# czbiohub-sf/shrimPy

Hardware: AMD Instinct MI355X
Metric: voxels/sec deskew+20-iter RL deconv, 2048×2048×512 f32; HBM GB/s vs peak (higher is better)
Workload: dtype f32

## Files before the change

### shrimpy_amd/csrc/rl_fused_sep.hip

```cpp

#include "common.hpp"
#include "correlate_common.hpp"

#ifndef LSR_FUSED_PZ
#error "compile with -DLSR_FUSED_PZ=<odd tap count along z>"
#endif

namespace {

using lsr::FusedArgs;

constexpr int kTX = lsr::kSepWideTileX;
constexpr int kWaves = 8;
constexpr int kThreads = 64 * kWaves;
constexpr int kBand = 8;
constexpr int kRing = 3;

constexpr int cdiv(int a, int b) { return (a + b - 1) / b; }

template <int PZ, int PYX, int RUN>
struct Geo {
  static constexpr int C = PYX / 2, CZ = PZ / 2;
  static constexpr int TY = 8 * RUN;
  static constexpr int WL = lsr::fused_window_halo(PYX);
  static constexpr int AR = TY + 4 * C;
  static constexpr int PA = kTX + 2 * WL;
  static constexpr int CH = PA / 4;
  static constexpr int NCH = AR * CH;
  static constexpr int SL = cdiv(NCH, kThreads);
  static constexpr int ASZ = cdiv(NCH, 64) * 64 * 4;
  static constexpr int NP = cdiv(4 + 2 * C, 4);
  static constexpr int G1 = (kTX + WL) / 4;
  static constexpr int PB1 = 4 * G1;
  static constexpr int NIT1 = AR * G1;
  static constexpr int XIT1 = cdiv(NIT1, kThreads);
  static constexpr int R1 = TY + 2 * C;
  static constexpr int RUN1 = cdiv(R1, 8);
  static constexpr int E = PB1 - kTX;
  static constexpr int NE = R1 * E;
  static constexpr int EP = cdiv(NE, kThreads);
  static constexpr int SH = WL - 2 * C;
  static constexpr int PR = 4 * (kTX / 4 - 1 + NP);
  static constexpr int RSZ = 4 + 8 * RUN1 * PR;
  static constexpr int NIT2 = R1 * (kTX / 4);
  static constexpr int XIT2 = cdiv(NIT2, kThreads);
  static constexpr int B1SZ = AR * PB1;
  static constexpr int B2SZ = R1 * kTX;
  static constexpr int OFF_B1 = kRing * ASZ;
  static constexpr int OFF_R = OFF_B1 + B1SZ;
  static constexpr int OFF_B2 = OFF_R + RSZ;
  static constexpr int OFF_DUMP = OFF_B2 + B2SZ;
  static constexpr int OFF_RNY = OFF_DUMP + 256;
  static constexpr int TOTAL = OFF_RNY + 32;
  static constexpr int NY = 2 * RUN1 + EP;
#ifdef LSR_FUSED_PROBE_NOXC
  static constexpr int NXC = 0;
#else
  static constexpr int NXC = 2 * RUN + 1;
#endif
  static_assert(TOTAL * 4 <= 160 * 1024, "LDS per workgroup");
  static_assert(PR == PB1, "B1 and R share a pitch");
  static_assert(2 * C <= WL && WL <= lsr::kSepOriginCol, "halo columns");
  static_assert(SL + 2 * (NY + NXC) <= 63, "vmcnt is a 6-bit counter");
  static_assert(OFF_B1 % 4 == 0 && OFF_R % 4 == 0 && OFF_B2 % 4 == 0, "16-byte aligned buffers");
};

typedef float f32x4 __attribute__((ext_vector_type(4)));
typedef float f32x2 __attribute__((ext_vector_type(2)));

__device__ __forceinline__ float fast_rcp(float d) {
  float r = __builtin_amdgcn_rcpf(d);
  return fmaf(fmaf(-d, r, 1.0f), r, r);
}
__device__ __forceinline__ f32x2 splat(float a) { return f32x2{a, a}; }
__device__ __forceinline__ f32x2 pk_fma(f32x2 a, f32x2 b, f32x2 c) { return __builtin_elementwise_fma(a, b, c); }
__device__ __forceinline__ f32x2 fast_rcp2(f32x2 d) {
  const f32x2 r = f32x2{__builtin_amdgcn_rcpf(d.x), __builtin_amdgcn_rcpf(d.y)};
  return pk_fma(pk_fma(-d, r, splat(1.0f)), r, r);
}
template <int PX, int NP>
__device__ __forceinline__ f32x4 xpass_item(const f32x4* src, const float (&wx)[PX]) {
  float w[4 * NP];
#pragma unroll
  for (int i = 0; i < NP; ++i) {
    const f32x4 v = src[i];
    w[4 * i] = v.x; w[4 * i + 1] = v.y; w[4 * i + 2] = v.z; w[4 * i + 3] = v.w;
  }
  f32x2 o01 = splat(wx[0]) * f32x2{w[0], w[1]};
  f32x2 o23 = splat(wx[0]) * f32x2{w[2], w[3]};
#pragma unroll
  for (int c = 1; c < PX; ++c) {
    o01 = pk_fma(splat(wx[c]), f32x2{w[c], w[c + 1]}, o01);
    o23 = pk_fma(splat(wx[c]), f32x2{w[c + 2], w[c + 3]}, o23);
  }
  return f32x4{o01.x, o01.y, o23.x, o23.y};
}

template <int IMM>
__device__ __forceinline__ void gload(float& dst, const float* sbase, int voff) {
  asm volatile("global_load_dword %0, %1, %2 offset:%3" : "+v"(dst) : "v"(voff), "s"(sbase), "n"(IMM) : "memory");
}
#ifndef LSR_FUSED_STORE_POLICY
#define LSR_FUSED_STORE_POLICY "nt"
#endif
#ifndef LSR_FUSED_GLDS_POLICY
#define LSR_FUSED_GLDS_POLICY ""
#endif
template <int IMM>
__device__ __forceinline__ void gstore(float* sbase, int voff, float v) {
  asm volatile("global_store_dword %0, %1, %2 offset:%3 " LSR_FUSED_STORE_POLICY
               :
               : "v"(voff), "v"(v), "s"(sbase), "n"(IMM)
               : "memory");
}
__device__ __forceinline__ void glds_x4(const float* sbase, int voff, unsigned lds_byte_addr) {
  asm volatile("s_mov_b32 m0, %2\n\ts_nop 0\n\tglobal_load_lds_dwordx4 %0, %1 " LSR_FUSED_GLDS_POLICY
               :
               : "v"(voff), "s"(sbase), "s"(lds_byte_addr)
               : "memory");
}
template <int N>
__device__ __forceinline__ void wait_vm() {
  asm volatile("s_waitcnt vmcnt(%0)" : : "n"(N) : "memory");
}
template <int K>
__device__ __forceinline__ void tie(float (&a)[K]) {
#pragma unroll
  for (int i = 0; i < K; ++i) asm volatile("" : "+v"(a[i]));
}
__device__ __forceinline__ void tie(float& a) { asm volatile("" : "+v"(a)); }
__device__ __forceinline__ void lds_barrier() {
  asm volatile("s_waitcnt lgkmcnt(0)" ::: "memory");
  __builtin_amdgcn_s_barrier();
  __builtin_amdgcn_sched_barrier(0);
}

template <int PZ, int PYX, int RUN, bool STATS>
__global__ __launch_bounds__(kThreads) void rl_fused_sep_kernel(FusedArgs p) {
  using T = Geo<PZ, PYX, RUN>;
  constexpr int C = T::C, CZ = T::CZ, TY = T::TY, RUN1 = T::RUN1, EP = T::EP;
  constexpr int NP = T::NP, NY = T::NY, NXC = T::NXC, SL = T::SL;
  __shared__ f32x4 smem4[T::TOTAL / 4];
  float* const smem = reinterpret_cast<float*>(smem4);
  f32x4* const B1_4 = smem4 + T::OFF_B1 / 4;
  const float* const B1 = smem + T::OFF_B1;
  float* const Rw = smem + T::OFF_R + 4;
  const f32x4* const R_4 = smem4 + T::OFF_R / 4 + 1;
  f32x4* const B2_4 = smem4 + T::OFF_B2 / 4;
  const float* const B2 = smem + T::OFF_B2;
  const unsigned lds_base =
      static_cast<unsigned>(reinterpret_cast<size_t>((__attribute__((address_space(3))) char*)smem4));

  const int tid = threadIdx.x;
  const int lane = tid & 63;
  const int wave = __builtin_amdgcn_readfirstlane(tid >> 6);

  auto xcd_contiguous = [](int b, int n) {
#ifdef LSR_FUSED_PLAIN_ORDER
    return b;
#endif
    const int per = n / 8, rem = n % 8;
    const int xcd = b % 8, idx = b / 8;
    return xcd * per + (xcd < rem ? xcd : rem) + idx;
  };
  const int Z = p.Z, Y = p.Y, X = p.X;
  int lin, zb, ze;
  if (static_cast<int>(blockIdx.x) < p.n_full) {
    lin = xcd_contiguous(blockIdx.x, p.n_full);
    zb = 0;
    ze = Z;
  } else {
    const int t = xcd_contiguous(blockIdx.x - p.n_full, gridDim.x - p.n_full);
    const int col = t / p.pieces;
    lin = p.n_full + col;
    zb = (t - col * p.pieces) * p.z_chunk;
    ze = min(zb + p.z_chunk, Z);
  }
  const int band = lin / (p.tiles_x * kBand);
  const int lb = lin - band * (p.tiles_x * kBand);
  const int band_h = min(kBand, p.tiles_y - band * kBand);
#if defined(LSR_FUSED_PLAIN_ORDER) && LSR_FUSED_PLAIN_ORDER == 2
  const int tx = lin % p.tiles_x;
  const int ty = lin / p.tiles_x;
  (void)lb; (void)band_h;
#else
  const int tx = lb / band_h;
  const int ty = band * kBand + (lb - tx * band_h);
#endif
  const int x0 = tx * kTX, y0 = ty * TY;
#ifdef LSR_FUSED_LAG
  if ((tx + ty) & 1) {
#pragma unroll
    for (int i = 0; i < LSR_FUSED_LAG; ++i) __builtin_amdgcn_s_sleep(127);
  }
#endif

  float tv0 = p.taps[lane], tv1 = p.taps[64 + (lane & 31)];
  auto load_taps = [&](int row, auto& w) {
#pragma unroll
    for (int i = 0; i < static_cast<int>(sizeof(w) / sizeof(float)); ++i) {
      const int f = row * 16 + i;
      w[i] = __int_as_float(__builtin_amdgcn_readlane(__float_as_int(f < 64 ? tv0 : tv1), f & 63));
    }
  };

  const float* const x_tile = p.x + (static_cast<int64_t>(y0 - 2 * C) * p.pitch + (x0 - T::WL));
  int s_voff[SL];
#pragma unroll
  for (int k = 0; k < SL; ++k) {
    const int e = min(tid + k * kThreads, T::NCH - 1);
    const int r = e / T::CH, c = e - r * T::CH;
    s_voff[k] = (r * p.pitch + 4 * c) * 4;
  }
  int a1_chunk[T::XIT1];
#pragma unroll
  for (int k = 0; k < T::XIT1; ++k) {
    const int i = min(tid + k * kThreads, T::NIT1 - 1);
    const int row = i / T::G1;
    a1_chunk[k] = i + row * (T::CH - T::G1);
  }
  const int r1_row0 = wave * RUN1;
  const int y1_col = r1_row0 * T::PB1 + lane;
  const int r_col = r1_row0 * T::PR + lane - T::SH;
  const bool interior = x0 - C >= 0 && x0 + kTX + C <= X && y0 - C >= 0 && y0 + TY + C <= Y;
  int e_b1[EP], e_voff[EP];
  int e_rc[EP];
#pragma unroll
  for (int e = 0; e < EP; ++e) {
    const int t = min(tid + e * kThreads, T::NE - 1);
    const int er = t / T::E, ec = t - er * T::E;
    e_b1[e] = er * T::PB1 + kTX + ec;
    e_rc[e] = (er << 16) | (kTX + ec);
    e_voff[e] = (er * p.y_pitch + kTX + ec) * 4;
  }
  const int y2_col = (wave * RUN) * kTX + lane;
  int xc_voff[RUN], o_voff[RUN], y_voff[RUN1];
#pragma unroll
  for (int m = 0; m < RUN; ++m) {
    xc_voff[m] = ((wave * RUN + m) * p.pitch + lane) * 4;
    o_voff[m] = ((wave * RUN + m) * p.out_pitch + lane) * 4;
  }
#pragma unroll
  for (int m = 0; m < RUN1; ++m) y_voff[m] = (min(r1_row0 + m, T::R1 - 1) * p.y_pitch + lane) * 4;
  float rnx[2];
#pragma unroll
  for (int cg = 0; cg < 2; ++cg) rnx[cg] = fast_rcp(p.nx[min(x0 + lane + 64 * cg, X - 1)]);
  float* const rny_lds = smem + T::OFF_RNY;
  if (tid < TY) rny_lds[tid] = fast_rcp(p.ny[min(y0 + tid, Y - 1)]);

  f32x2 acc1[PZ][RUN1], acc2[PZ][RUN];
  float acc1e[PZ][EP];
#pragma unroll
  for (int j = 0; j < PZ; ++j) {
#pragma unroll
    for (int i = 0; i < RUN1; ++i) acc1[j][i] = splat(0.0f);
#pragma unroll
    for (int i = 0; i < EP; ++i) acc1e[j][i] = 0.0f;
#pragma unroll
    for (int i = 0; i < RUN; ++i) acc2[j][i] = splat(0.0f);
  }
  float yv[2 * RUN1], ye[EP], xc[2 * RUN], nzv = 1.0f;
#pragma unroll
  for (int i = 0; i < 2 * RUN1; ++i) yv[i] = 0.0f;
#pragma unroll
  for (int i = 0; i < EP; ++i) ye[i] = 0.0f;
#pragma unroll
  for (int i = 0; i < 2 * RUN; ++i) xc[i] = 0.0f;
  const f32x2 rnx2 = f32x2{rnx[0], rnx[1]};
  f32x2 st_flux = splat(0.0f), st_total = splat(0.0f);
  float st_change = 0.0f;
  auto st_add = [&](f32x2 x_old, f32x2 xu, f32x2 v) {
    st_flux += xu;
    st_total += v;
    const f32x2 d = v - x_old;
    st_change += __builtin_fabsf(d.x);
    st_change += __builtin_fabsf(d.y);
  };
  __builtin_amdgcn_sched_barrier(0);

  auto clampz = [&](int z) { return min(max(z, 0), Z - 1); };
  auto issue_glds = [&](int plane, int slot) {
    const float* src = x_tile + static_cast<int64_t>(clampz(plane)) * p.plane;
    const unsigned dst = lds_base + (slot * T::ASZ + wave * 64 * 4) * 4;
#pragma unroll
    for (int k = 0; k < SL; ++k) {
      const bool live = wave * 64 + k * kThreads < T::NCH;
      glds_x4(src, s_voff[k], live ? dst + k * kThreads * 16 : lds_base + T::OFF_DUMP * 4);
    }
  };
  const float* const xc_tile = p.x + (static_cast<int64_t>(y0) * p.pitch + x0);
  const float* const y_tile = p.y + (static_cast<int64_t>(y0 - C) * p.y_pitch + (x0 + C - T::WL));
  float* const o_tile = p.out + (static_cast<int64_t>(y0) * p.out_pitch + x0);
  auto issue_xc = [&](int o) {
#ifdef LSR_FUSED_PROBE_NOXC
    return;
#endif
    const int oc = clampz(o);
    const float* base = xc_tile + static_cast<int64_t>(oc) * p.plane;
#pragma unroll
    for (int m = 0; m < RUN; ++m) {
      gload<0>(xc[m], base, xc_voff[m]);
      gload<256>(xc[RUN + m], base, xc_voff[m]);
    }
    gload<0>(nzv, p.nz + oc, 0);
  };
  auto issue_y = [&](int q) {
    const float* base = y_tile + static_cast<int64_t>(clampz(q)) * p.y_plane;
#pragma unroll
    for (int m = 0; m < RUN1; ++m) {
      gload<0>(yv[m], base, y_voff[m]);
      gload<256>(yv[RUN1 + m], base, y_voff[m]);
    }
#pragma unroll
    for (int e = 0; e < EP; ++e) gload<0>(ye[e], base, e_voff[e]);
  };

  const int q_lo = max(zb - CZ, 0), q_hi = min(ze - 1 + CZ, Z - 1);
  const int p_lo = max(q_lo - CZ, 0);
  const int p_hi = ze + 2 * CZ;

  int slot = 0;
  issue_glds(p_lo, 0);
  issue_xc(p_lo - 1 - 2 * CZ);
  issue_y(p_lo - CZ);
  issue_glds(p_lo + 1, 1);
  issue_xc(p_lo - 1 - 2 * CZ);
  issue_y(p_lo - CZ);
  wait_vm<SL + 2 * (NXC + NY)>();
  lds_barrier();

#ifdef LSR_FUSED_PROBE_TIME
  if (p.probe && tid == 0) p.probe[4 * blockIdx.x] = wall_clock64();
#endif
  for (int pz = p_lo; pz <= p_hi; ++pz) {
    asm volatile("" : "+v"(tv0), "+v"(tv1));
#ifdef LSR_FUSED_PROBE_TIME
    if (p.probe && tid == 0 && (pz == p_lo + 40 || pz == p_lo + 120))
      p.probe[4 * blockIdx.x + (pz == p_lo + 40 ? 1 : 2)] = wall_clock64();
#endif
    const int qr = pz - 1 - CZ;
    const int o = qr - CZ;
    const int q = pz - CZ;
    const bool x_live = pz < Z && pz <= q_hi + CZ;
    const bool r_live = qr >= q_lo && qr <= q_hi;
    const int slot2 = slot >= 1 ? slot - 1 : 2;

    issue_glds(pz + 2, slot2);
#ifdef LSR_FUSED_PROBE_NOCOMPUTE
    if (false) {
#else
    if (x_live) {
#endif
      float w1x[PYX];
      load_taps(0, w1x);
      const f32x4* A_4 = smem4 + slot * (T::ASZ / 4);
#pragma unroll
      for (int k = 0; k < T::XIT1; ++k)
        if (k + 1 < T::XIT1 || tid + k * kThreads < T::NIT1)
          B1_4[tid + k * kThreads] = xpass_item<PYX, NP>(A_4 + a1_chunk[k], w1x);
    } else {
#pragma unroll
      for (int k = 0; k < T::XIT1; ++k)
        if (k + 1 < T::XIT1 || tid + k * kThreads < T::NIT1) B1_4[tid + k * kThreads] = f32x4{0, 0, 0, 0};
    }
#ifdef LSR_FUSED_PROBE_NOCOMPUTE
    if (false) {
#else
    if (r_live) {
#endif
      float w2x[PYX];
      load_taps(3, w2x);
#pragma unroll
      for (int k = 0; k < T::XIT2; ++k) {
        const int j = tid + k * kThreads;
        if (k + 1 < T::XIT2 || j < T::NIT2)
          B2_4[j] = xpass_item<PYX, NP>(R_4 + (j + (j >> 5) * (T::PR / 4 - kTX / 4)), w2x);
      }
    } else {
#pragma unroll
      for (int k = 0; k < T::XIT2; ++k)
        if (k + 1 < T::XIT2 || tid + k * kThreads < T::NIT2) B2_4[tid + k * kThreads] = f32x4{0, 0, 0, 0};
    }
    lds_barrier();

    {
      float w2y[PYX], w2z[PZ];
      load_taps(4, w2y);
      load_taps(5, w2z);
      f32x2 pl[RUN];
#ifdef LSR_FUSED_PROBE_NOCOMPUTE
#pragma unroll
      for (int m = 0; m < RUN; ++m) pl[m] = splat(B2[y2_col + m]);
      if (false)
#endif
      {
        const float* colp = B2 + y2_col;
        f32x2 cv[RUN + 2 * C];
#pragma unroll
        for (int j = 0; j < RUN + 2 * C; ++j) cv[j] = f32x2{colp[j * kTX], colp[j * kTX + 64]};
#pragma unroll
        for (int m = 0; m < RUN; ++m) {
          f32x2 s2 = splat(w2y[0]) * cv[m];
#pragma unroll
          for (int b = 1; b < PYX; ++b) s2 = pk_fma(splat(w2y[b]), cv[m + b], s2);
          pl[m] = s2;
        }
      }
#pragma unroll
      for (int j = 0; j < PZ - 1; ++j)
#pragma unroll
        for (int i = 0; i < RUN; ++i) acc2[j][i] = pk_fma(splat(w2z[PZ - 1 - j]), pl[i], acc2[j + 1][i]);
#pragma unroll
      for (int i = 0; i < RUN; ++i) acc2[PZ - 1][i] = splat(w2z[0]) * pl[i];

      wait_vm<NY + SL>();
      tie(xc);
      tie(nzv);
#ifdef LSR_FUSED_PROBE_NOSTORE
      if (o >= zb && o < ze && nzv == 12345.678f) {
#else
      if (o >= zb && o < ze) {
#endif
        float* obase = o_tile + static_cast<int64_t>(o) * p.out_plane;
        const float rz = fast_rcp(nzv);
        if (!p.mask_out) {
#pragma unroll
          for (int m = 0; m < RUN; ++m) {
            const f32x2 xo = f32x2{xc[m], xc[RUN + m]};
            const f32x2 xu = xo * acc2[0][m];
            const f32x2 v = xu * (splat(rz * rny_lds[wave * RUN + m]) * rnx2);
            gstore<0>(obase, o_voff[m], v.x);
            gstore<256>(obase, o_voff[m], v.y);
            if constexpr (STATS) st_add(xo, xu, v);
          }
        } else {
          const bool ok0 = x0 + lane < X, ok1 = x0 + lane + 64 < X;
#pragma unroll
          for (int m = 0; m < RUN; ++m) {
            if (y0 + wave * RUN + m < Y) {
              const f32x2 xo = f32x2{xc[m], xc[RUN + m]};
              const f32x2 xu = xo * acc2[0][m];
              const f32x2 v = xu * (splat(rz * rny_lds[wave * RUN + m]) * rnx2);
              if (ok0) gstore<0>(obase, o_voff[m], v.x);
              if (ok1) gstore<256>(obase, o_voff[m], v.y);
              if constexpr (STATS) {
                st_add(xo, xu, v);
              }
            }
          }
        }
      }
      __builtin_amdgcn_sched_barrier(0);
      issue_xc(o + 1);
    }
    {
      float w1y[PYX], w1z[PZ];
      load_taps(1, w1y);
      load_taps(2, w1z);
      f32x2 pl[RUN1];
      float ple[EP];
#ifdef LSR_FUSED_PROBE_NOCOMPUTE
#pragma unroll
      for (int m = 0; m < RUN1; ++m) pl[m] = splat(B1[y1_col + m]);
      if (false)
#endif
      {
        const float* colp = B1 + y1_col;
        f32x2 cv[RUN1 + 2 * C];
#pragma unroll
        for (int j = 0; j < RUN1 + 2 * C; ++j) cv[j] = f32x2{colp[j * T::PB1], colp[j * T::PB1 + 64]};
#pragma unroll
        for (int m = 0; m < RUN1; ++m) {
          f32x2 s2 = splat(w1y[0]) * cv[m];
#pragma unroll
          for (int b = 1; b < PYX; ++b) s2 = pk_fma(splat(w1y[b]), cv[m + b], s2);
          pl[m] = s2;
        }
      }
#pragma unroll
      for (int e = 0; e < EP; ++e) {
        const float* colp = B1 + e_b1[e];
#ifdef LSR_FUSED_PROBE_NOCOMPUTE
        ple[e] = colp[0];
        continue;
#endif
        float s1 = w1y[0] * colp[0];
#pragma unroll
        for (int b = 1; b < PYX; ++b) s1 = fmaf(w1y[b], colp[b * T::PB1], s1);
        ple[e] = s1;
      }
#pragma unroll
      for (int j = 0; j < PZ - 1; ++j) {
#pragma unroll
        for (int i = 0; i < RUN1; ++i) acc1[j][i] = pk_fma(splat(w1z[PZ - 1 - j]), pl[i], acc1[j + 1][i]);
#pragma unroll
        for (int e = 0; e < EP; ++e) acc1e[j][e] = fmaf(w1z[PZ - 1 - j], ple[e], acc1e[j + 1][e]);
      }
#pragma unroll
      for (int i = 0; i < RUN1; ++i) acc1[PZ - 1][i] = splat(w1z[0]) * pl[i];
#pragma unroll
      for (int e = 0; e < EP; ++e) acc1e[PZ - 1][e] = w1z[0] * ple[e];

      wait_vm<SL + NXC>();
      tie(yv);
      tie(ye);
      const bool q_in = q >= q_lo && q <= q_hi;
      if (q_in && interior) {
#pragma unroll
        for (int m = 0; m < RUN1; ++m) {
          const f32x2 r = f32x2{yv[m], yv[RUN1 + m]} * fast_rcp2(acc1[0][m] + splat(p.eps));
          Rw[r_col + m * T::PR] = r.x;
          Rw[r_col + m * T::PR + 64] = r.y;
        }
#pragma unroll
        for (int e = 0; e < EP; ++e)
          if (e + 1 < EP || tid + e * kThreads < T::NE)
            Rw[e_b1[e] - T::SH] = ye[e] * fast_rcp(acc1e[0][e] + p.eps);
      } else {
        const int gx0 = x0 + lane + C - T::WL;
        const bool in0 = q_in && gx0 >= 0 && gx0 < X, in1 = q_in && gx0 + 64 >= 0 && gx0 + 64 < X;
#pragma unroll
        for (int m = 0; m < RUN1; ++m) {
          const int gy = y0 + r1_row0 + m - C;
          const bool row_in = gy >= 0 && gy < Y && r1_row0 + m < T::R1;
          const f32x2 r = f32x2{yv[m], yv[RUN1 + m]} * fast_rcp2(acc1[0][m] + splat(p.eps));
          Rw[r_col + m * T::PR] = (row_in && in0) ? r.x : 0.0f;
          Rw[r_col + m * T::PR + 64] = (row_in && in1) ? r.y : 0.0f;
        }
#pragma unroll
        for (int e = 0; e < EP; ++e) {
          if (e + 1 < EP || tid + e * kThreads < T::NE) {
            const int gy = y0 + (e_rc[e] >> 16) - C, gx = x0 + (e_rc[e] & 0xffff) + C - T::WL;
            const float r = ye[e] * fast_rcp(acc1e[0][e] + p.eps);
            Rw[e_b1[e] - T::SH] = (q_in && gy >= 0 && gy < Y && gx >= 0 && gx < X) ? r : 0.0f;
          }
        }
      }
      __builtin_amdgcn_sched_barrier(0);
      issue_y(q + 1);
    }
    wait_vm<SL + 2 * (NXC + NY)>();
    lds_barrier();
    slot = slot == 2 ? 0 : slot + 1;
  }
  asm volatile("s_waitcnt vmcnt(0)" ::: "memory");
  if constexpr (STATS) {
    lsr::keep_until_here(xc);
    lsr::keep_until_here(yv);
    lsr::keep_until_here(ye);
    lsr::keep_until_here(nzv);
    asm volatile("" : "+v"(st_flux), "+v"(st_total), "+v"(st_change));
    lsr::RlStats st;
    st.flux = st_flux.x + st_flux.y;
    st.change = st_change;
    st.total = st_total.x + st_total.y;
    lsr::rl_stats_flush<kWaves>(st, smem + T::OFF_B2, p.stats);
  }
#ifdef LSR_FUSED_PROBE_TIME
  if (p.probe && tid == 0) p.probe[4 * blockIdx.x + 3] = wall_clock64();
#endif
}

template <int PZ, int PYX>
bool launch_one(const FusedArgs& p, dim3 grid, hipStream_t s) {
  if constexpr (lsr::fused_compiled(PZ, PYX)) {
    constexpr int RUN = lsr::fused_run(PZ, PYX);
    if (p.stats != nullptr) hipLaunchKernelGGL((rl_fused_sep_kernel<PZ, PYX, RUN, true>), grid, dim3(kThreads), 0, s, p);
    else hipLaunchKernelGGL((rl_fused_sep_kernel<PZ, PYX, RUN, false>), grid, dim3(kThreads), 0, s, p);
    return true;
  } else {
    return false;
  }
}

}

namespace lsr {

#define LSR_CAT2(a, b) a##b
#define LSR_CAT(a, b) LSR_CAT2(a, b)
bool LSR_CAT(launch_fused_pz, LSR_FUSED_PZ)(int pyx, const FusedArgs& p, unsigned blocks, hipStream_t s) {
  constexpr int PZ = LSR_FUSED_PZ;
  const dim3 grid(blocks);
  switch (pyx) {
    case 3: return launch_one<PZ, 3>(p, grid, s);
    case 5: return launch_one<PZ, 5>(p, grid, s);
    case 7: return launch_one<PZ, 7>(p, grid, s);
    case 9: return launch_one<PZ, 9>(p, grid, s);
    case 11: return launch_one<PZ, 11>(p, grid, s);
    case 13: return launch_one<PZ, 13>(p, grid, s);
    case 15: return launch_one<PZ, 15>(p, grid, s);
    default: return false;
  }
}

}
```

Before: 41.27 billion.

## Load filter taps via scalar constant loads and specialize mask path at compile time

Replaces the per-lane tap vectors fetched with readlane by scalar loads through the constant address space. This frees two VGPRs per thread and moves tap fetches to the scalar unit, with the loads hoisted before the LDS barriers so their latency overlaps. The mask_out branch becomes a template parameter, removing a runtime branch and doubling the number of kernel instantiations. The glds liveness check is also simplified so only the last chunk is predicated.

```diff
diff --git a/shrimpy_amd/csrc/rl_fused_sep.hip b/shrimpy_amd/csrc/rl_fused_sep.hip
--- a/shrimpy_amd/csrc/rl_fused_sep.hip
+++ b/shrimpy_amd/csrc/rl_fused_sep.hip
@@ -135,7 +135,7 @@
   __builtin_amdgcn_sched_barrier(0);
 }
 
-template <int PZ, int PYX, int RUN, bool STATS>
+template <int PZ, int PYX, int RUN, bool STATS, bool MASK>
 __global__ __launch_bounds__(kThreads) void rl_fused_sep_kernel(FusedArgs p) {
   using T = Geo<PZ, PYX, RUN>;
   constexpr int C = T::C, CZ = T::CZ, TY = T::TY, RUN1 = T::RUN1, EP = T::EP;
@@ -195,13 +195,12 @@
   }
 #endif
 
-  float tv0 = p.taps[lane], tv1 = p.taps[64 + (lane & 31)];
+  typedef const __attribute__((address_space(4))) float* ctaps_t;
+  const float* taps = p.taps;
   auto load_taps = [&](int row, auto& w) {
-#pragma unroll
-    for (int i = 0; i < static_cast<int>(sizeof(w) / sizeof(float)); ++i) {
-      const int f = row * 16 + i;
-      w[i] = __int_as_float(__builtin_amdgcn_readlane(__float_as_int(f < 64 ? tv0 : tv1), f & 63));
-    }
+    const ctaps_t t = (ctaps_t)taps;
+#pragma unroll
+    for (int i = 0; i < static_cast<int>(sizeof(w) / sizeof(float)); ++i) w[i] = t[row * 16 + i];
   };
 
   const float* const x_tile = p.x + (static_cast<int64_t>(y0 - 2 * C) * p.pitch + (x0 - T::WL));
@@ -284,7 +283,7 @@
     const unsigned dst = lds_base + (slot * T::ASZ + wave * 64 * 4) * 4;
 #pragma unroll
     for (int k = 0; k < SL; ++k) {
-      const bool live = wave * 64 + k * kThreads < T::NCH;
+      const bool live = k + 1 < SL || wave * 64 + k * kThreads < T::NCH;
       glds_x4(src, s_voff[k], live ? dst + k * kThreads * 16 : lds_base + T::OFF_DUMP * 4);
     }
   };
@@ -332,8 +331,11 @@
 #ifdef LSR_FUSED_PROBE_TIME
   if (p.probe && tid == 0) p.probe[4 * blockIdx.x] = wall_clock64();
 #endif
+  float w1x[PYX], w2x[PYX];
+  load_taps(0, w1x);
+  load_taps(3, w2x);
   for (int pz = p_lo; pz <= p_hi; ++pz) {
-    asm volatile("" : "+v"(tv0), "+v"(tv1));
+    asm volatile("" : "+s"(taps));
 #ifdef LSR_FUSED_PROBE_TIME
     if (p.probe && tid == 0 && (pz == p_lo + 40 || pz == p_lo + 120))
       p.probe[4 * blockIdx.x + (pz == p_lo + 40 ? 1 : 2)] = wall_clock64();
@@ -351,8 +353,6 @@
 #else
     if (x_live) {
 #endif
-      float w1x[PYX];
-      load_taps(0, w1x);
       const f32x4* A_4 = smem4 + slot * (T::ASZ / 4);
 #pragma unroll
       for (int k = 0; k < T::XIT1; ++k)
@@ -368,8 +368,6 @@
 #else
     if (r_live) {
 #endif
-      float w2x[PYX];
-      load_taps(3, w2x);
 #pragma unroll
       for (int k = 0; k < T::XIT2; ++k) {
         const int j = tid + k * kThreads;
@@ -381,12 +379,14 @@
       for (int k = 0; k < T::XIT2; ++k)
         if (k + 1 < T::XIT2 || tid + k * kThreads < T::NIT2) B2_4[tid + k * kThreads] = f32x4{0, 0, 0, 0};
     }
+    float w2y[PYX], w2z[PZ], w1y[PYX], w1z[PZ];
+    load_taps(4, w2y);
+    load_taps(5, w2z);
+    load_taps(1, w1y);
+    load_taps(2, w1z);
     lds_barrier();
 
     {
-      float w2y[PYX], w2z[PZ];
-      load_taps(4, w2y);
-      load_taps(5, w2z);
       f32x2 pl[RUN];
 #ifdef LSR_FUSED_PROBE_NOCOMPUTE
 #pragma unroll
@@ -423,7 +423,7 @@
 #endif
         float* obase = o_tile + static_cast<int64_t>(o) * p.out_plane;
         const float rz = fast_rcp(nzv);
-        if (!p.mask_out) {
+        if constexpr (!MASK) {
 #pragma unroll
           for (int m = 0; m < RUN; ++m) {
             const f32x2 xo = f32x2{xc[m], xc[RUN + m]};
@@ -454,9 +454,6 @@
       issue_xc(o + 1);
     }
     {
-      float w1y[PYX], w1z[PZ];
-      load_taps(1, w1y);
-      load_taps(2, w1z);
       f32x2 pl[RUN1];
       float ple[EP];
 #ifdef LSR_FUSED_PROBE_NOCOMPUTE
@@ -540,6 +537,8 @@
       issue_y(q + 1);
     }
     wait_vm<SL + 2 * (NXC + NY)>();
+    load_taps(0, w1x);
+    load_taps(3, w2x);
     lds_barrier();
     slot = slot == 2 ? 0 : slot + 1;
   }
@@ -561,12 +560,18 @@
 #endif
 }
 
+template <int PZ, int PYX, bool STATS>
+void launch_stats(const FusedArgs& p, dim3 grid, hipStream_t s) {
+  constexpr int RUN = lsr::fused_run(PZ, PYX);
+  if (p.mask_out) hipLaunchKernelGGL((rl_fused_sep_kernel<PZ, PYX, RUN, STATS, true>), grid, dim3(kThreads), 0, s, p);
+  else hipLaunchKernelGGL((rl_fused_sep_kernel<PZ, PYX, RUN, STATS, false>), grid, dim3(kThreads), 0, s, p);
+}
+
 template <int PZ, int PYX>
 bool launch_one(const FusedArgs& p, dim3 grid, hipStream_t s) {
   if constexpr (lsr::fused_compiled(PZ, PYX)) {
-    constexpr int RUN = lsr::fused_run(PZ, PYX);
-    if (p.stats != nullptr) hipLaunchKernelGGL((rl_fused_sep_kernel<PZ, PYX, RUN, true>), grid, dim3(kThreads), 0, s, p);
-    else hipLaunchKernelGGL((rl_fused_sep_kernel<PZ, PYX, RUN, false>), grid, dim3(kThreads), 0, s, p);
+    if (p.stats != nullptr) launch_stats<PZ, PYX, true>(p, grid, s);
+    else launch_stats<PZ, PYX, false>(p, grid, s);
     return true;
   } else {
     return false;
```

After: 41.11 billion, median of 2. About the same (-0.4%).
